# VISION-SJTU/UniDefense

Hardware: AMD Instinct MI355X
Metric: images/sec fwd+bwd (256x256, EffNet-b4) (higher is better)
Workload: dtype f32

## Files before the change

### include/unidefense_hip.h

```cpp
#ifndef UNIDEFENSE_HIP_H
#define UNIDEFENSE_HIP_H
#include <stdint.h>

#ifdef __cplusplus
extern "C" {
#endif

#define UD_EINVAL (-1000)

typedef void* ud_stream_t;

typedef struct {
    int N, Hin, Win, Cin, Hout, Wout, KH, KW, stride, pad_t, pad_l, transposed;
} ud_conv_geom;

typedef struct {
    const float* A; const float* B; float* C;
    int M, N, K;
    long lda, ldb, ldc;
    int a_mode, b_mode, out_mode, split_k;
    int batch; long strideA, strideB, strideC;
    ud_conv_geom g;
    double* stat_sum; double* stat_sumsq;
    int half_mask;
// ... 363 lines not shown
int ud_pw_bwd_fused_ok(int CE, int CIN);
int ud_pw_bwd_set_form(int form);
long ud_pw_bwd_fused_grid(long M);
int ud_pw_bwd_fused(const float* e, const float* dz, const ud_bn_ref* bn, const double* s1, const double* s2,
                    const double* s1_local, const double* s2_local, const float* x, const float* w, const float* add, long M,
                    int CE, int CIN, float* dx, float* dw, float* part, float* dgamma, float* dbeta, ud_stream_t stream);
int ud_pj_bwd_fused_ok(int CE, int CO, int HW);
int ud_pj_fwd_fused_ok(int CE, int CO, int HW);
int ud_pj_fwd_fused(const float* d, const ud_bn_ref* bn, const float* s, const float* w, int N, int HW, int CE, int CO, float* p,
                    double* sum, double* sumsq, ud_stream_t stream);
long ud_pj_bwd_fused_grid(int N, int HW, int CE, int CO);
int ud_mb_eval_dw_ok(int Ci, int CE, int K, int stride);
long ud_mb_eval_dw_tiles(int Ho, int Wo, int stride);
int ud_mb_eval_dw(const float* x, const float* we, const ud_bn_ref* bn0, const float* wt, const ud_bn_ref* bn1, float* d, float* part,
                  int N, int H, int W, int Ci, int CE, int Ho, int Wo, int K, int stride, int pad_t, int pad_l, int out_act,
                  ud_stream_t stream);
int ud_mb_eval_dw_h_ok(int Ci, int CE, int K, int stride);
long ud_mb_eval_dw_h_tiles(int Ho, int Wo, int stride);
int ud_mb_eval_dw_h(const void* x, const float* we, const ud_bn_ref* bn0, const float* wt, const ud_bn_ref* bn1, void* d, float* part,
                    int N, int H, int W, int Ci, int CE, int Ho, int Wo, int K, int stride, int pad_t, int pad_l, int out_act,
                    ud_stream_t stream);
int ud_pj_bwd_fused_a(const float* d, const float* dp, const ud_bn_ref* bn, const float* s, const float* w, int N, int HW, int CE,
                      int CO, float* dw, double* dgate, float* part, ud_stream_t stream);
int ud_pj_bwd_fused_b(const float* d, const float* dp, const ud_bn_ref* bn, const float* s, const float* dpool, float inv_hw,
                      const float* w, int N, int HW, int CE, int CO, float* dz, double* s1, double* s2, ud_stream_t stream);
int ud_normbwd_apply_plane_half(const void* x, const void* dy, const float* keep, float inv_keep, const ud_bn_ref* bn,
                                int dy_is_dz, const double* s1, const double* s2, const double* s1_local,
                                const double* s2_local, int G, int R, int C, uint16_t* plane, long panel_stride,
                                float* inv_scale, float* dgamma, float* dbeta, ud_stream_t stream);
int ud_se_bwd_a(const double* dgate, const float* s2, const float* s1, const float* We, double* ds1_acc, float* dWe,
                float* dbe, int N, int C, int Cs, ud_stream_t stream);
int ud_se_bwd_b(const double* ds1_acc, const float* s1, const float* Wr, const double* pool, float pool_scale,
                float* dpool, float* dWr, float* dbr, int N, int C, int Cs, ud_stream_t stream);
int ud_se_scale_bwd_bn(const void* dc, const void* x, const ud_bn_ref* bn, const float* s, const float* dpool,
    float inv_hw, void* dz, double* s1, double* s2, double* ws, int G, int R, int C, int f16, ud_stream_t
    stream);
long ud_coldot_bn_eval_ws_doubles(int G, int R, int C);
int ud_coldot_bn_eval(const void* dy, const void* x, const ud_bn_ref* bn, int G, int R, int C, double* out, double* ws,
                      int f16, ud_stream_t stream);
int ud_se_scale_bwd_bn_eval(const void* dc, const void* x, const ud_bn_ref* bn, const float* s, const float* dpool,
                            float inv_hw, void* dd, int G, int R, int C, int f16, ud_stream_t stream);
int ud_bn_eval_bwd(const void* dy, const void* x, const ud_bn_ref* bn, void* dx, int G, int R, int C, int f16,
                   ud_stream_t stream);
int ud_normbwd_apply_mix(const void* x, const void* dz, const ud_bn_ref* bn, const double* s1, const double* s2,
    const double* s1_local, const double* s2_local, const void* diff, int G, int R, int C, void* dd,
    double* dalpha_acc, float* dgamma, float* dbeta, double* energy, int f16, ud_stream_t stream);
int ud_gate_grad_from_acc(const double* acc, const float* alpha, float* out, ud_stream_t stream);
int ud_bn_apply(const void* x, const ud_bn_ref* bn, void* y, int G, int R, int C, int f16, ud_stream_t stream);
int ud_dwconv_bwd_data_bn(const void* dy, const float* gate_alpha, int gate_mode, const float* wt, const void*
    add, const void* x, const ud_bn_ref* bn, void* dz, double* s1, double* s2, double* ws, int N, int H, int W,
    int C, int Ho, int Wo, int K, int stride, int pad_t, int pad_l, int f16, ud_stream_t stream);
long ud_dwconv_bwd_data_bn_ws_doubles(int N, int H, int W, int C, int stride);
int ud_dwconv_bwd_data_ex(const void* dy, const float* gate_alpha, int gate_mode, const float* wt, const void*
    add, void* dx, int N, int H, int W, int C, int Ho, int Wo, int K, int stride, int pad_t, int pad_l, int f16,
    ud_stream_t stream);
int ud_dwconv_bwd_weight_ex(const void* x, const void* dy, const float* gate_alpha, int gate_mode, float* dwt,
    float* part, int chunks, int N, int H, int W, int C, int Ho, int Wo, int K, int stride, int pad_t, int
    pad_l, int f16, ud_stream_t stream);
int ud_rfft2_ex(const void* x, void* Y, int N, int S, int C, float scale, float w_interior, const ud_bn_ref* bn,
    void* act_out, const float* gate_alpha, int gate_mode, const double* gate_acc, float* gate_grad, int f16,
    uint32_t* absmax, ud_stream_t stream);
int ud_rfft2_ex_planes(const void* x, uint16_t* planes, long panel_stride, long plane_stride, float* inv_scale, float bound_pre,
                       const double* energy, int N, int S, int C, float scale, float w_interior, const ud_bn_ref* bn,
                       void* act_out, const float* gate_alpha, int gate_mode, const double* gate_acc, float* gate_grad,
                       const float* dw_wt, void* dw_out, int dw_k, ud_stream_t stream);
int ud_irfft2_mix(const void* Y, void* y, int N, int S, int C, float scale, float w_interior, const void* spat,
// ... 65 lines not shown
```

### unidefense_amd/csrc/fused.hip

```cpp
#include "bnref.h"

namespace {

struct Rows {
    int r, r_end;
    long idx, step;
};
__device__ __forceinline__ Rows rows_of(const RedGeom& q, int ri, int c4) {
    Rows w;
    const int g = blockIdx.z, p = blockIdx.x;
    const int r_begin = p * q.rows_per_chunk;
    w.r_end = r_begin + q.rows_per_chunk;
    if (w.r_end > q.R) w.r_end = q.R;
    w.step = (long)q.rpi * q.C4;
    w.r = r_begin + ri;
    w.idx = (long)g * q.R * q.C4 + (long)w.r * q.C4 + c4;
    return w;
}

__device__ __forceinline__ bool is_updater(int ri) { return blockIdx.x == 0 && blockIdx.z == 0 && ri == 0; }

template <int NQ>
__device__ __forceinline__ void red_out(const RedGeom& q, int ri, bool active, int c4, double (&v)[8], double* a1,
                                        double* a2, double* part, bool per_group) {
// ... 1217 lines not shown
                       (const _Float16*)nullptr, (_Float16*)nullptr, (double*)nullptr, dgamma, dbeta, (uint32_t*)nullptr,
                       (double*)nullptr, PlanesDst{plane, panel_stride, 0, inv_scale, nullptr});
    UD_LAUNCH_CHECK();
    return 0;
}

int ud_normbwd_apply_mix(const void* x, const void* dz, const ud_bn_ref* bn, const double* s1, const double* s2,
                         const double* s1_local, const double* s2_local, const void* diff, int G, int R, int C,
                         void* dd, double* dalpha_acc, float* dgamma, float* dbeta, double* energy, int f16,
                         ud_stream_t stream) {
    if (ud_bn_eval_form(bn)) return UD_EINVAL;
    if (!shape_ok(G, R, C) || !x || !dz || !bn || !s1 || !s2 || !dd || !diff || !dalpha_acc || bn->G != 1)
        return UD_EINVAL;
    if ((dgamma || dbeta) && (!s1_local || !s2_local)) return UD_EINVAL;
    RedGeom q = make_geom_ex(G, R, C, 512, 4096, 4);
    UD_STORAGE_DISPATCH(f16, hipLaunchKernelGGL((normbwd_apply_kernel<T, true>), red_grid(q), dim3(NT), 0,
                                                (hipStream_t)stream, q, (const T*)x, (const T*)dz, (const float*)nullptr,
                                                1.f, *bn, 1, s1, s2, s1_local, s2_local, (const T*)diff, (T*)dd,
                                                dalpha_acc, dgamma, dbeta, (uint32_t*)nullptr, energy,
                                                PlanesDst{nullptr, 0, 0, nullptr, nullptr}));
    UD_LAUNCH_CHECK();
    return 0;
}

int ud_gate_grad_from_acc(const double* acc, const float* alpha, float* out, ud_stream_t stream) {
    if (!acc || !alpha || !out) return UD_EINVAL;
    hipLaunchKernelGGL(gate_grad_from_acc_kernel, dim3(1), dim3(64), 0, (hipStream_t)stream, acc, alpha, out);
    UD_LAUNCH_CHECK();
    return 0;
}

int ud_se_bwd_a(const double* dgate, const float* s2, const float* s1, const float* We, double* ds1_acc, float* dWe,
                float* dbe, int N, int C, int Cs, ud_stream_t stream) {
    if (N < 1 || C < 1 || Cs < 1 || Cs > 128 || !dgate || !s2 || !s1 || !We || !ds1_acc || (!dWe != !dbe)) return UD_EINVAL;
    hipStream_t s = (hipStream_t)stream;
    const int role1 = N * ud_cdiv(C, Cs <= 64 ? 32 * (NT / 64) : 32 * (NT / 128));
    const bool wg = dWe != nullptr;
    if (Cs <= 64) {
        dim3 grid((unsigned)(role1 + (wg ? ud_cdiv(C, NT / 64) : 0)));
        hipLaunchKernelGGL(se_bwd_a_kernel<64>, grid, dim3(NT), 0, s, dgate, s2, s1, We, ds1_acc, dWe, dbe, N, C, Cs);
    } else {
        dim3 grid((unsigned)(role1 + (wg ? ud_cdiv(C, NT / 128) : 0)));
        hipLaunchKernelGGL(se_bwd_a_kernel<128>, grid, dim3(NT), 0, s, dgate, s2, s1, We, ds1_acc, dWe, dbe, N, C, Cs);
    }
    UD_LAUNCH_CHECK();
    return 0;
}

int ud_se_bwd_b(const double* ds1_acc, const float* s1, const float* Wr, const double* pool, float pool_scale,
                float* dpool, float* dWr, float* dbr, int N, int C, int Cs, ud_stream_t stream) {
    const bool wg = dWr != nullptr;
    if (N < 1 || N > NT || C < 1 || Cs < 1 || Cs > NT || !ds1_acc || !s1 || !Wr || !dpool || (!dWr != !dbr) || (wg && !pool))
        return UD_EINVAL;
    dim3 grid((unsigned)ud_cdiv(C, NT), (unsigned)(N + (wg ? Cs : 0)));
    hipLaunchKernelGGL(se_bwd_b_kernel, grid, dim3(NT), 0, (hipStream_t)stream, ds1_acc, s1, Wr, pool, pool_scale, dpool,
                       dWr, dbr, N, C, Cs);
    UD_LAUNCH_CHECK();
    return 0;
}

int ud_se_scale_bwd_bn(const void* dc, const void* x, const ud_bn_ref* bn, const float* s, const float* dpool,
                       float inv_hw, void* dz, double* s1, double* s2, double* ws, int G, int R, int C, int f16,
                       ud_stream_t stream) {
    if (ud_bn_eval_form(bn)) return UD_EINVAL;
    if (!shape_ok(G, R, C) || !dc || !x || !bn || !s || !dpool || !dz || !s1 || !s2 || bn->G != 1) return UD_EINVAL;
    hipStream_t st = (hipStream_t)stream;
    RedPlan pl = plan_reduce(G, R, C, false, ws);
    UD_STORAGE_DISPATCH(f16, hipLaunchKernelGGL(se_scale_bwd_bn_kernel<T>, red_grid(pl.q), dim3(NT), 0, st, pl.q,
                                                (const T*)dc, (const T*)x, *bn, s, dpool, inv_hw, (T*)dz, s1, s2,
                                                pl.use_part ? ws : nullptr));
    UD_LAUNCH_CHECK();
    return finish_reduce(pl, 2, false, C, ws, s1, s2, st);
}

static RedGeom coldot_eval_geom(int G, int R, int C) { return make_geom_ex(G, R, C, 1024, 64, 8); }

long ud_coldot_bn_eval_ws_doubles(int G, int R, int C) {
// ... 144 lines not shown
```

### unidefense_amd/kernels.py

```python
import ctypes as C
import math
import os

import torch

from . import lib as _lib
from .config import cfg as CFG
from .devmem import Scratch, ZeroPool
from .lib import ConvGeom, GemmDesc, GemmP3Desc

_call = _lib.call
_const, _rows = _lib.const, _lib.const_rows

GEMM_PROFILE = None


def _stream():
    return C.c_void_p(torch.cuda.current_stream().cuda_stream)


def _p(t):
    if t is None:
        return None
    return C.c_void_p(t.data_ptr())
# ... 2591 lines not shown
def se_scale_bn_planes(x, bn, s, G, R, amax):
    _chk(x, s)
    Cc = x.shape[-1]
    pl = Planes(G * R, Cc, x, 2, False)
    _call("ud_se_scale_bn_planes", _p(x), C.byref(bn.ref()), _p(s), _p(pl.buf), pl.panel, pl.plane, _p(pl.inv), _p(amax), G, R, Cc,
          _stream())
    return pl


def se_scale_bn_plane_half(x, bn, s, G, R):
    _act(x)
    _chk(s)
    Cc = x.shape[-1]
    pl = Planes(G * R, Cc, x, 1, False)
    _call("ud_se_scale_bn_plane_half", _p(x), C.byref(bn.ref()), _p(s), _p(pl.buf), pl.panel, _p(pl.inv), G, R, Cc, _stream())
    return pl


def coldot_bn(dy, x, bn, G, R, out):
    h = _act(dy, x)
    Cc = x.shape[-1]
    _call("ud_coldot_bn", _p(dy), _p(x), C.byref(bn.ref()), G, R, Cc, _pd(out), _fused_ws(x, G, R, Cc, True), h,
          _stream())


def fc_fwd_d(xsum, xscale, W, b, N):
    _chk(W, b)
    O, I = W.shape
    y = empty((N, O), W)
    _call("ud_fc_fwd_d", _pd(xsum), float(xscale), _p(W), _p(b), _p(y), N, I, O, _stream())
    return y


def bn_apply(x, bn, G, R, update=False):
    h = _act(x)
    y = torch.empty_like(x)
    _call("ud_bn_apply", _p(x), C.byref(bn.ref(update)), _p(y), G, R, x.shape[-1], h, _stream())
    return y


def se_scale_bn(x, bn, s, G, R, want_absmax=False):
    h = _act(x)
    _chk(s)
    y = torch.empty_like(x)
    amax = amax_slots(x, want_absmax)
    _call("ud_se_scale_bn", _p(x), C.byref(bn.ref()), _p(s), _p(y), G, R, x.shape[-1], h, _p(amax), _stream())
    y._ud_absmax = amax
    return y


def residual_bn(x, bn, keep, inv_keep, skip, G, R, update=False, want_absmax=False, planes_for=None):
    h = _act(x, skip)
    _chk(keep)
    out = torch.empty_like(x)
    amax = amax_slots(x, want_absmax)
    Cc = x.shape[-1]
    skip_amax = getattr(skip, "_ud_absmax", None) if skip is not None else None
    if (planes_for is not None and h == 0 and Cc % 4 == 0 and CFG.spectral_p2 != "off"
            and (skip is None or skip_amax is not None)
            and spectral_takes_planes(planes_for[0], planes_for[1], Cc, planes_for[2], want_stats=True)):
        pl = Planes(G * R, Cc, x, 2, False)
        _call("ud_residual_bn_planes", _p(x), C.byref(bn.ref(update)), _p(keep), float(inv_keep), _p(skip), _p(skip_amax), _p(out),
              _p(pl.buf), pl.panel, pl.plane, _p(pl.inv), G, R, Cc, _p(amax), _stream())
        out._ud_planes = pl
    else:
        _call("ud_residual_bn", _p(x), C.byref(bn.ref(update)), _p(keep), float(inv_keep), _p(skip), _p(out), G, R,
# ... 114 lines not shown


def project_bwd_fused_b(d, bn, s, dpool, inv_hw, dp2, w2, N, HW, sacc):
    _chk(d, dp2, w2, s, dpool)
    Co, Ce = w2.shape
    dz = torch.empty_like(d)
    _call("ud_pj_bwd_fused_b", _p(d), _p(dp2), C.byref(bn.ref()), _p(s), _p(dpool), float(inv_hw), _p(w2), N, HW, Ce, Co, _p(dz),
          _pd(sacc), _pd(sacc, Ce), _stream())
    return dz


def normbwd_apply_mix(x, dz, bn, G, R, sacc, diff, dalpha_acc, sacc_local=None, energy=None):
    h = _act(x, dz, diff)
    Cc = x.shape[-1]
    loc = sacc if sacc_local is None else sacc_local
    dd = torch.empty_like(x)
    dg = empty((Cc,), x)
    db = empty((Cc,), x)
    _call("ud_normbwd_apply_mix", _p(x), _p(dz), C.byref(bn.ref()), _pd(sacc), _pd(sacc, Cc), _pd(loc), _pd(loc, Cc),
          _p(diff), G, R, Cc, _p(dd), _pd(dalpha_acc), _p(dg), _p(db), _pd(energy) if energy is not None else None, h, _stream())
    return dd, dg, db


def gate_grad_from_acc(acc, alpha):
    out = empty((), alpha)
    _call("ud_gate_grad_from_acc", _pd(acc), _p(alpha), _p(out), _stream())
    return out


def se_bwd(dgate, s2, s1, We, Wr, pool, pool_scale, need_w=True):
    _chk(s2, s1, We, Wr)
    N, Cc = s2.shape
    Cs = s1.shape[1]
    ds1_acc = zeros64(N * Cs, s2)
    if not need_w:
        _call("ud_se_bwd_a", _pd(dgate), _p(s2), _p(s1), _p(We), _pd(ds1_acc), None, None, N, Cc, Cs, _stream())
        dpool = empty((N, Cc), s2)
        _call("ud_se_bwd_b", _pd(ds1_acc), _p(s1), _p(Wr), None, 0.0, _p(dpool), None, None, N, Cc, Cs, _stream())
        return dpool, None, None, None, None
    dWe = empty((Cc, Cs), s2)
    dbe = empty((Cc,), s2)
    _call("ud_se_bwd_a", _pd(dgate), _p(s2), _p(s1), _p(We), _pd(ds1_acc), _p(dWe), _p(dbe), N, Cc, Cs, _stream())
    dpool = empty((N, Cc), s2)
    dWr = empty((Cs, Cc), s2)
    dbr = empty((Cs,), s2)
    _call("ud_se_bwd_b", _pd(ds1_acc), _p(s1), _p(Wr), _pd(pool), float(pool_scale), _p(dpool), _p(dWr), _p(dbr), N, Cc,
          Cs, _stream())
    return dpool, dWe, dbe, dWr, dbr


def se_scale_bwd_bn(dc, x, bn, s, dpool, inv_hw, G, R, sacc):
    h = _act(dc, x)
    _chk(s, dpool)
    Cc = x.shape[-1]
    dz = torch.empty_like(x)
    _call("ud_se_scale_bwd_bn", _p(dc), _p(x), C.byref(bn.ref()), _p(s), _p(dpool), float(inv_hw), _p(dz), _pd(sacc),
          _pd(sacc, Cc), _fused_ws(x, G, R, Cc, False), G, R, Cc, h, _stream())
    return dz


def coldot_bn_eval(dy, x, bn, G, R, out):
    h = _act(dy, x)
    Cc = x.shape[-1]
    ws = _ws64(x, _call("ud_coldot_bn_eval_ws_doubles", G, R, Cc))
    _call("ud_coldot_bn_eval", _p(dy), _p(x), C.byref(bn.ref()), G, R, Cc, _pd(out), ws, h, _stream())

# ... 302 lines not shown
```

### unidefense_amd/mbconv.py

```python
import collections
from types import SimpleNamespace

import torch

from . import kernels as K
from . import tape as T
from .config import cfg


FUSED, HALF, EVAL_NODE, OPERATORS = "fused", "half", "eval_node", "operators"
TrunkMode = collections.namedtuple("TrunkMode", "kind wt dp", defaults=(None,))


_DW_TILED = True


_DW_TILE_OVERRIDE = {}
_DW_BWD_FUSED_OVERRIDE = {}


def _dw_tile_policy(sf, k, stride, H, half):
    ov = _DW_TILE_OVERRIDE.get((bool(sf), k, stride, H, bool(half)))
    if ov is not None and _DW_TILED:
        return ov
# ... 200 lines not shown
    if spat is None and t_fwd:
        spat = K.dwtile_fwd(src, wt, k, g.pt, g.pl, g.Ho, g.Wo, bn=src_bn, stride=stride)
    elif spat is None:
        spat = K.dwconv_fwd(a, wt, k, stride, g.pt, g.pl, g.Ho, g.Wo)
    b.a = a
    b.xf_shape = (g.N, S, S // 2 + 1, 2 * Ce)
    if isinstance(xf, K.Planes):
        yf, b.sctx = K.spectral_fwd(xf, g.Wf)
    else:
        yf, b.sctx = K.spectral_fwd(xf.view(-1, 2 * Ce), g.Wf, x_absmax=getattr(xf, "_ud_absmax", None))
    yf = yf.view(b.xf_shape)
    xf = None
    if stride == 1:
        b.d, b.fr = K.irfft2_mix(yf, g.s_i, spat, g.alpha, acc1)
        spat = None
    else:
        b.fr = K.irfft2(yf, g.s_i, 1.0)
        b.d = K.sfmix_fwd(spat, b.fr, g.alpha, True)
        K.colstats(b.d.view(g.Mo, Ce), acc1)
        b.spat = spat
    del yf


def _fwd_se(b):
    g, x, blk, d = b.geo, b.x, b.blk, b.d
    b.pool = K.zeros64(g.N * g.Ce, x)
    b.c_pl = (d.dtype == torch.float32 and g.Ce % 32 == 0 and cfg.spectral_p2 != "off"
              and K.spectral_takes_planes(g.Mo, g.Co, g.Ce, g.Wp, want_stats=True))
    c_amax = None
    if b.c_pl:
        c_amax = K.colsum_bn_amax(d, b.bn1, g.N, g.HWo, b.pool, update=True)
    else:
        K.colsum_bn(d, b.bn1, g.N, g.HWo, b.pool, update=True)
    b.s1 = K.fc_fwd_d(b.pool, 1.0 / g.HWo, g.Wsr, blk._se_reduce.bias, g.N)
    b.s2 = K.fc_fwd(b.s1, g.Wse, blk._se_expand.bias, 1)
    return c_amax


def _fwd_project(b, c_amax, next_blk):
    g, x, blk, d, bn1, s2 = b.geo, b.x, b.blk, b.d, b.bn1, b.s2
    acc2 = K.zeros64(2 * g.Co, x)
    if not b.c_pl and K.project_fwd_fused_ok(d, g.Wp, g.HWo):
        p, b.pctx = K.project_fwd_fused(d, bn1, s2, g.Wp, g.N, g.HWo, stats=acc2)
        done = True
    elif b.c_pl:
        c = K.se_scale_bn_planes(d, bn1, s2, g.N, g.HWo, c_amax)
        (p, done), b.pctx = K.spectral_fwd(c, g.Wp, stats=acc2)
    elif (d.dtype == torch.float16 and g.Ce % 8 == 0 and K.spectral_takes_plane_half(g.Mo, g.Co, g.Ce)):
        c = K.se_scale_bn_plane_half(d, bn1, s2, g.N, g.HWo)
        (p, done), b.pctx = K.spectral_fwd(c, g.Wp, stats=acc2)
    else:
        c = K.se_scale_bn(d, bn1, s2, g.N, g.HWo, want_absmax=True)
        (p, done), b.pctx = K.spectral_fwd(c.view(g.Mo, g.Ce), g.Wp, stats=acc2, x_absmax=getattr(c, "_ud_absmax", None))
    if not done:
        K.colstats(p, acc2)
    b.dp.reduce(acc2)
    b.bn2 = _bn_of(blk._bn2, acc2, g.Mo * b.dp.world, 0)
    b.p4 = p.view(g.N, g.Ho, g.Wo, g.Co)
    nxt = None
    if next_blk is not None and next_blk.spec.expand != 1:
        nxt = (g.Mo, next_blk.spec.cexp, next_blk._expand_conv.weight.view(next_blk.spec.cexp, g.Co))
    b.out = K.residual_bn(b.p4, b.bn2, b.keep, b.inv_keep, x if blk.spec.skip else None, g.N, g.HWo, update=True, want_absmax=True, planes_for=nxt)


def _fused_backward(b, tape):
    dout = tape.pop_grad(b.out)
    if dout is None:
        return
# ... 142 lines not shown
    if thin:
        dx, dWe, dg0, db0 = _expand_dgrad(tape, skip, dout, x, lambda acc: K.expand_bwd_fused(e, dz0, b.bn0, sb0, loc0, ectx.x, ectx.w, add=acc))
    else:
        de2, de_amax, dg0, db0 = _normbwd_to_gemm(ectx, gr.de_pl, e, dz0, None, 1.0, b.bn0, gr.is_dz, 1, g.M, sb0, loc0)
    tape.add_param_grad(blk._bn0.weight, dg0)
    tape.add_param_grad(blk._bn0.bias, db0)
    if not thin:
        dx, dWe = _expand_dgrad(tape, skip, dout, x, lambda acc: K.spectral_bwd(ectx, de2, out=acc, dy_absmax=de_amax))
    tape.add_param_grad(blk._expand_conv.weight, dWe)
    return dx


def _half_forward(x, blk, g, wt, src_bn):
    bn1 = K.EvalBN(blk._bn1, 1)
    if g.We is not None:
        src, src_bn = K.gemm_nt(x.view(g.M, g.Cin), g.We).view(g.N, g.H, g.W, g.Ce), K.EvalBN(blk._bn0, 1)
    else:
        src = x
    spat = K.dwtile_fwd(src, wt, g.k, g.pt, g.pl, g.Ho, g.Wo, bn=src_bn, stride=g.stride)
    xf_shape = None
    if g.sf:
        xf, _ = K.rfft2_ex(src, g.s_f, 1.0, bn=src_bn)
        xf_shape = xf.shape
        yf = K.gemm_nt(xf.view(-1, 2 * g.Ce), g.Wf).view(xf_shape)
        if g.stride == 1:
            d, _ = K.irfft2_mix(yf, g.s_i, spat, g.alpha, None)
        else:
            d = K.sfmix_fwd(spat, K.irfft2(yf, g.s_i, 1.0), g.alpha, True)
        del xf, yf, spat
    else:
        d = spat
    pool = K.zeros64(g.N * g.Ce, x)
    K.colsum_bn(d, bn1, g.N, g.HWo, pool)
    s1 = K.fc_fwd_d(pool, 1.0 / g.HWo, g.Wsr, blk._se_reduce.bias, g.N)
    out, s2, bn2 = _eval_half_tail(x, blk, g, d, bn1, s1)
    return out, SimpleNamespace(src=src, src_bn=src_bn, d=d, s1=s1, s2=s2, bn1=bn1, bn2=bn2, xf_shape=xf_shape)


def _eval_half_tail(x, blk, g, d, bn1, s1):
    s2 = K.fc_fwd(s1, g.Wse, blk._se_expand.bias, 1)
    p = K.gemm_nt(K.se_scale_bn(d, bn1, s2, g.N, g.HWo).view(g.Mo, g.Ce), g.Wp)
    bn2 = K.EvalBN(blk._bn2, 0)
    return K.residual_bn(p.view(g.N, g.Ho, g.Wo, g.Co), bn2, None, 1.0, x if blk.spec.skip else None, g.N, g.HWo), s2, bn2


def mbconv_eval_half(x, blk, wt, lazy_bn=None, node_max_cin=0):
    sp = blk.spec
    g = block_geom(blk, x)
    assert x.dtype == torch.float16 and not (sp.skip and lazy_bn is not None)
    if (sp.expand != 1 and sp.sf_norm is None and g.Cin <= node_max_cin and K.mb_eval_dw_h_ok(g.Cin, g.Ce, g.k, g.stride)):
        bn1 = K.EvalBN(blk._bn1, 1)
        d, pmean = K.mb_eval_dw_h(x, g.We, K.EvalBN(blk._bn0, 1), wt, bn1, g.k, g.stride, g.pt, g.pl, g.Ho, g.Wo, out_act=False)
        s1 = K.fc_fwd(pmean, g.Wsr, blk._se_reduce.bias, 0)
        return _eval_half_tail(x, blk, g, d, bn1, s1)[0]
    return _half_forward(x, blk, g, wt, lazy_bn)[0]


HALF_GRAD_PROBE = None


def mbconv_frozen_half(tape, x, blk, wt, lazy_in=None):
    if tape.wgrad_on:
        raise RuntimeError("mbconv_frozen_half is the backward of a FROZEN model (no parameter requires a gradient): it forms no "
                           "weight gradient; a half-storage backward with trainable parameters is the training step's")
    assert x.dtype == torch.float16 and not (blk.spec.skip and lazy_in is not None)
    g = block_geom(blk, x)
    out, f = _half_forward(x, blk, g, wt, lazy_in.bn if lazy_in is not None else None)
    tape.record(lambda: _frozen_backward(tape, x, blk, g, wt, lazy_in, out, f))
    return out


def _frozen_backward(tape, x, blk, g, wt, lazy_in, out, f):
    dout = tape.pop_grad(out)
    if dout is None:
        return
    dout = _grad_like(dout, out)
    assert dout.dtype == torch.float16
    skip, d, N, HWo = blk.spec.skip, f.d, g.N, g.HWo
    probe = HALF_GRAD_PROBE
    dp = K.bn_eval_bwd(dout, None, f.bn2, 1, g.Mo)
    dc = K.gemm_nn(dp.view(g.Mo, g.Co), g.Wp).view(N, g.Ho, g.Wo, g.Ce)
    if probe is not None:
        for nm, t in (("dout", dout), ("dp", dp), ("dc", dc)):
            probe(blk, nm, t)
    dgate = K.zeros64(N * g.Ce, x)
    K.coldot_bn_eval(dc, d, f.bn1, N, HWo, dgate)
    dpool = K.se_bwd(dgate, f.s2, f.s1, g.Wse, g.Wsr, None, 1.0 / HWo, need_w=False)[0]
# ... 11 lines not shown
            for nm, t in (("dyf", dyf), ("dxf", dxf), ("da_f", da_f)):
                probe(blk, nm, t)
        del dfr, dyf, dxf
        g_alpha, g_mode = g.alpha, 2
    if f.src_bn is not None:
        de = K.dwtile_dgrad_eval(dd, wt, g.k, g.pt, g.pl, f.src, f.src_bn, g_alpha, g_mode, da_f, g.stride)
        if probe is not None:
            probe(blk, "de", de)
        if lazy_in is not None:
            lazy_in.backward(de)
            return
        dx, = _expand_dgrad(tape, skip, dout, x, lambda acc: (K.gemm_nn(de.view(g.M, g.Ce), g.We, out=acc, accumulate=acc is not None),))
    else:
        add, skip_done = _skip_into_add(skip, da_f, dout)
        dx = K.dwtile_bwd_data(dd, wt, g.k, g.pt, g.pl, g.H, g.W, g_alpha, g_mode, add, stride=g.stride)
        if not skip_done:
            dx = K.axpby(dx, 1.0, dout, 1.0, out=dx)
    if probe is not None:
        probe(blk, "dx", dx)
    dx._ud_owned = True
    tape.add_grad(x, dx)


def eval_block_ok(blk, max_cin):
    sp = blk.spec
    return (sp.expand != 1 and sp.sf_norm is None and sp.cin <= max_cin and K.mb_eval_dw_ok(sp.cin, sp.cexp, sp.k, sp.stride))


def mbconv_eval(x, blk, wt):
    g = block_geom(blk, x)
    bn1 = K.EvalBN(blk._bn1, 1)
    pj = K.project_fwd_fused_ok(x, g.Wp, g.HWo)
    d, pool = K.mb_eval_dw(x, g.We, K.EvalBN(blk._bn0, 1), wt, bn1, g.k, g.stride, g.pt, g.pl, g.Ho, g.Wo, out_act=not pj)
    s1 = K.fc_fwd(pool, g.Wsr, blk._se_reduce.bias, 0)
    s2 = K.fc_fwd(s1, g.Wse, blk._se_expand.bias, 1)
    if pj:
        p, _ = K.project_fwd_fused(d, bn1, s2, g.Wp, g.N, g.HWo)
    else:
        p = K.gemm_nt(K.se_scale_fwd(d, s2).view(g.Mo, g.Ce), g.Wp)
    return K.residual_bn(p.view(g.N, g.Ho, g.Wo, g.Co), K.EvalBN(blk._bn2, 0), None, 1.0, x if blk.spec.skip else None, g.N, g.HWo)
```

Measured before the change: 1439.

## Fuse SE reduce/expand FCs into one kernel forward and one kernel backward

Adds a fused squeeze-excite kernel that runs the reduce FC, swish and expand FC in a single launch, keeping the pooled vector and hidden activations in LDS. A fused backward kernel computes dpool and all four weight and bias gradients in one multi-role launch, replacing the two-stage ud_se_bwd_a/ud_se_bwd_b path and its float64 accumulation buffer. The aim is to cut launch count and the global round trips for the small SE tensors in every MBConv block. Each path is gated by size heuristics on C*Cs and N*C and falls back to the old kernels otherwise. The generalised se_bwd_a template for Cs above 128 adds code paths with little coverage.

```diff
diff --git a/include/unidefense_hip.h b/include/unidefense_hip.h
--- a/include/unidefense_hip.h
+++ b/include/unidefense_hip.h
@@ -419,6 +419,13 @@
                 float* dbe, int N, int C, int Cs, ud_stream_t stream);
 int ud_se_bwd_b(const double* ds1_acc, const float* s1, const float* Wr, const double* pool, float pool_scale,
                 float* dpool, float* dWr, float* dbr, int N, int C, int Cs, ud_stream_t stream);
+#define UD_SE_FC_MAX_C 4096
+#define UD_SE_FC_MAX_CS 128
+int ud_se_fc_fwd(const double* pool_sum, float pool_scale, const float* pool_mean, const float* Wr, const float* br,
+                 const float* We, const float* be, float* s1, float* s2, int N, int C, int Cs, ud_stream_t stream);
+int ud_se_fc_bwd(const double* dgate, const float* s2, const float* s1, const float* We, const float* Wr,
+                 const double* pool, float pool_scale, float* dpool, float* dWe, float* dbe, float* dWr, float* dbr, int N,
+                 int C, int Cs, ud_stream_t stream);
 int ud_se_scale_bwd_bn(const void* dc, const void* x, const ud_bn_ref* bn, const float* s, const float* dpool,
     float inv_hw, void* dz, double* s1, double* s2, double* ws, int G, int R, int C, int f16, ud_stream_t
     stream);
diff --git a/unidefense_amd/csrc/fused.hip b/unidefense_amd/csrc/fused.hip
--- a/unidefense_amd/csrc/fused.hip
+++ b/unidefense_amd/csrc/fused.hip
@@ -1273,17 +1273,18 @@
 
 int ud_se_bwd_a(const double* dgate, const float* s2, const float* s1, const float* We, double* ds1_acc, float* dWe,
                 float* dbe, int N, int C, int Cs, ud_stream_t stream) {
-    if (N < 1 || C < 1 || Cs < 1 || Cs > 128 || !dgate || !s2 || !s1 || !We || !ds1_acc || (!dWe != !dbe)) return UD_EINVAL;
+    if (N < 1 || C < 1 || Cs < 1 || Cs > NT || !dgate || !s2 || !s1 || !We || !ds1_acc || (!dWe != !dbe)) return UD_EINVAL;
     hipStream_t s = (hipStream_t)stream;
-    const int role1 = N * ud_cdiv(C, Cs <= 64 ? 32 * (NT / 64) : 32 * (NT / 128));
+    const int ip = Cs <= 64 ? 64 : (Cs <= 128 ? 128 : NT);
+    const int role1 = N * ud_cdiv(C, 32 * (NT / ip));
     const bool wg = dWe != nullptr;
-    if (Cs <= 64) {
-        dim3 grid((unsigned)(role1 + (wg ? ud_cdiv(C, NT / 64) : 0)));
+    dim3 grid((unsigned)(role1 + (wg ? ud_cdiv(C, NT / ip) : 0)));
+    if (ip == 64)
         hipLaunchKernelGGL(se_bwd_a_kernel<64>, grid, dim3(NT), 0, s, dgate, s2, s1, We, ds1_acc, dWe, dbe, N, C, Cs);
-    } else {
-        dim3 grid((unsigned)(role1 + (wg ? ud_cdiv(C, NT / 128) : 0)));
+    else if (ip == 128)
         hipLaunchKernelGGL(se_bwd_a_kernel<128>, grid, dim3(NT), 0, s, dgate, s2, s1, We, ds1_acc, dWe, dbe, N, C, Cs);
-    }
+    else
+        hipLaunchKernelGGL(se_bwd_a_kernel<NT>, grid, dim3(NT), 0, s, dgate, s2, s1, We, ds1_acc, dWe, dbe, N, C, Cs);
     UD_LAUNCH_CHECK();
     return 0;
 }
diff --git a/unidefense_amd/csrc/sefc.hip b/unidefense_amd/csrc/sefc.hip
--- /dev/null
+++ b/unidefense_amd/csrc/sefc.hip
@@ -0,0 +1,387 @@
+#include "ud_common.h"
+
+namespace {
+
+constexpr int NTS = 1024;
+constexpr int NW = NTS / 64;
+constexpr int MAXC = UD_SE_FC_MAX_C;
+constexpr int MAXCS = UD_SE_FC_MAX_CS;
+constexpr int KU = 16;
+static_assert(MAXC % (64 * KU) == 0 && MAXCS <= NTS / 8, "the padded trip counts and the LDS carves below assume these");
+constexpr int KUR = 4;
+constexpr int RU = 2;
+constexpr int NR = 64;
+
+__device__ __forceinline__ float dpre_at(const double* dgate, const float* s2, long i) {
+    const float g = ud_sigmoid_fast(s2[i]);
+    return (float)dgate[i] * g * (1.f - g);
+}
+
+template <bool WAVE_OUT>
+__global__ __launch_bounds__(NTS) void se_fc_fwd_kernel(const double* __restrict__ xsum, float xscale,
+                                                        const float* __restrict__ xmean, const float* __restrict__ Wr,
+                                                        const float* __restrict__ br, const float* __restrict__ We,
+                                                        const float* __restrict__ be, float* __restrict__ s1,
+                                                        float* __restrict__ s2, int C, int Cs, int span) {
+    __shared__ float sx[MAXC];
+    __shared__ float sh[MAXCS];
+    const int n = blockIdx.y, tid = threadIdx.x, lane = tid & 63, wave = tid >> 6;
+    const int KP = ((C + 63) / 64 + KU - 1) / KU * KU;
+    for (int c = tid; c < KP * 64; c += NTS)
+        sx[c] = c < C ? (xsum ? (float)xsum[(long)n * C + c] * xscale : xmean[(long)n * C + c]) : 0.f;
+    __syncthreads();
+    for (int i = wave; i < Cs; i += 2 * NW) {
+        const bool two = i + NW < Cs;
+        const float* w0 = Wr + (long)i * C;
+        const float* w1 = Wr + (long)(two ? i + NW : i) * C;
+        float acc0 = 0.f, acc1 = 0.f;
+        for (int k0 = 0; k0 < KP; k0 += KU) {
+            float wv0[KU], wv1[KU];
+#pragma unroll
+            for (int j = 0; j < KU; ++j) {
+                const int cc = min(lane + 64 * (k0 + j), C - 1);
+                wv0[j] = w0[cc];
+                wv1[j] = w1[cc];
+            }
+#pragma unroll
+            for (int j = 0; j < KU; ++j) {
+                const float xv = sx[lane + 64 * (k0 + j)];
+                acc0 += xv * wv0[j];
+                acc1 += xv * wv1[j];
+            }
+        }
+        acc0 = ud_wave_sum(acc0);
+        acc1 = ud_wave_sum(acc1);
+        if (lane < 2 && (lane == 0 || two)) {
+            const int iu = i + lane * NW;
+            const float v = (lane ? acc1 : acc0) + (br ? br[iu] : 0.f);
+            sh[iu] = ud_swish(v);
+            if (blockIdx.x == 0) s1[(long)n * Cs + iu] = v;
+        }
+    }
+    __syncthreads();
+    const int o_end = min(C, ((int)blockIdx.x + 1) * span);
+    if (WAVE_OUT) {
+        for (int o = blockIdx.x * span + wave; o < o_end; o += NW) {
+            float acc = 0.f;
+#pragma unroll 4
+            for (int i = lane; i < Cs; i += 64) acc += sh[i] * We[(long)o * Cs + i];
+            acc = ud_wave_sum(acc);
+            if (lane == 0) s2[(long)n * C + o] = acc + (be ? be[o] : 0.f);
+        }
+        return;
+    }
+    for (int o = blockIdx.x * span + tid; o < o_end; o += NTS) {
+        const float* w = We + (long)o * Cs;
+        float acc = 0.f;
+        if ((Cs & 3) == 0) {
+#pragma unroll 8
+            for (int i = 0; i < Cs; i += 4) {
+                const f32x4 v = *reinterpret_cast<const f32x4*>(w + i);
+                acc += sh[i] * v[0] + sh[i + 1] * v[1] + sh[i + 2] * v[2] + sh[i + 3] * v[3];
+            }
+        } else {
+#pragma unroll 4
+            for (int i = 0; i < Cs; ++i) acc += sh[i] * w[i];
+        }
+        s2[(long)n * C + o] = acc + (be ? be[o] : 0.f);
+    }
+}
+
+constexpr int LDS_BWD = MAXC + 4 * NTS + 16 * MAXCS + MAXCS;
+
+__global__ __launch_bounds__(NTS) void se_fc_bwd_kernel(const double* __restrict__ dgate, const float* __restrict__ s2,
+                                                        const float* __restrict__ s1, const float* __restrict__ We,
+                                                        const float* __restrict__ Wr, const double* __restrict__ pool,
+                                                        float pool_scale, float* __restrict__ dpool,
+                                                        float* __restrict__ dWe, float* __restrict__ dbe,
+                                                        float* __restrict__ dWr, float* __restrict__ dbr, int N, int C,
+                                                        int Cs, int G, int span, int EB) {
+    __shared__ float lds[LDS_BWD];
+    const int tid = threadIdx.x, lane = tid & 63, wave = tid >> 6;
+    int b = blockIdx.x;
+    if (b < N * G) {
+        float* dp = lds;
+        float* part = lds + MAXC;
+        float* part2 = part + 4 * NTS;
+        float* ds = part2 + 16 * MAXCS;
+        const int n = b / G, g = b % G;
+        constexpr int PW = 8;
+        const int c0 = g * span, cn = min(span, C - c0);
+        const int SL = min(min(NTS / span, Cs), 16);
+        const int cl = tid % span, sl = tid / span;
+        const bool pooler = sl < SL && cl < cn, pre = (Cs + SL - 1) / SL <= PW;
+        const float s1v = tid < Cs ? s1[(long)n * Cs + tid] : 0.f;
+        float wv[PW];
+#pragma unroll
+        for (int j = 0; j < PW; ++j) {
+            const int i = sl + j * SL;
+            wv[j] = (pooler && pre && i < Cs) ? Wr[(long)i * C + c0 + cl] : 0.f;
+        }
+        for (int c = tid; c < C; c += NTS) dp[c] = dpre_at(dgate, s2, (long)n * C + c);
+        __syncthreads();
+        const int V = (Cs & 3) ? 1 : 4, Q = Cs / V, R = NTS / Q;
+        const int q = tid % Q, r = tid / Q;
+        if (r < R) {
+            const int TP = ((C + R - 1) / R + 7) / 8 * 8;
+            if (V == 4) {
+                f32x4 a = {0.f, 0.f, 0.f, 0.f};
+                for (int t0 = 0; t0 < TP; t0 += 8) {
+                    f32x4 v[8];
+                    float d[8];
+#pragma unroll
+                    for (int j = 0; j < 8; ++j) {
+                        const int c = r + (t0 + j) * R, cc = min(c, C - 1);
+                        v[j] = *reinterpret_cast<const f32x4*>(We + (long)cc * Cs + 4 * q);
+                        d[j] = c < C ? dp[cc] : 0.f;
+                    }
+#pragma unroll
+                    for (int j = 0; j < 8; ++j) a += d[j] * v[j];
+                }
+                *reinterpret_cast<f32x4*>(part + r * Cs + 4 * q) = a;
+            } else {
+                float a = 0.f;
+                for (int t0 = 0; t0 < TP; t0 += 8) {
+                    float v[8], d[8];
+#pragma unroll
+                    for (int j = 0; j < 8; ++j) {
+                        const int c = r + (t0 + j) * R, cc = min(c, C - 1);
+                        v[j] = We[(long)cc * Cs + q];
+                        d[j] = c < C ? dp[cc] : 0.f;
+                    }
+#pragma unroll
+                    for (int j = 0; j < 8; ++j) a += d[j] * v[j];
+                }
+                part[r * Cs + q] = a;
+            }
+        }
+        __syncthreads();
+        const int H = min(NTS / Cs, 16);
+        {
+            const int i = tid % Cs, h = tid / Cs;
+            if (h < H) {
+                float s = 0.f;
+                for (int rr = h; rr < R; rr += H) s += part[rr * Cs + i];
+                part2[h * Cs + i] = s;
+            }
+        }
+        __syncthreads();
+        if (tid < Cs) {
+            float s = 0.f;
+            for (int h = 0; h < H; ++h) s += part2[h * Cs + tid];
+            ds[tid] = s * ud_act_grad_fast(s1v, 1);
+        }
+        __syncthreads();
+        if (pooler) {
+            float a = 0.f;
+            if (pre) {
+#pragma unroll
+                for (int j = 0; j < PW; ++j) a += (sl + j * SL < Cs ? ds[sl + j * SL] : 0.f) * wv[j];
+            } else {
+                const float* w = Wr + c0 + cl;
+#pragma unroll 8
+                for (int i = sl; i < Cs; i += SL) a += ds[i] * w[(long)i * C];
+            }
+            part[sl * span + cl] = a;
+        }
+        __syncthreads();
+        if (tid < cn) {
+            float s = 0.f;
+            for (int k = 0; k < SL; ++k) s += part[k * span + tid];
+            dpool[(long)n * C + c0 + tid] = s;
+        }
+        return;
+    }
+    b -= N * G;
+    if (b < EB) {
+        float* sh = lds;
+        const int IP = Cs <= 64 ? 64 : 128, NSL = NTS / IP;
+        const int i = tid % IP, sl = tid / IP;
+        const int c = b * NSL + sl;
+        const bool own = c < C && i < Cs;
+        float acc = 0.f, accb = 0.f;
+        for (int n0 = 0; n0 < N; n0 += IP) {
+            const int nn = min(IP, N - n0);
+            __syncthreads();
+            sh[sl * IP + i] = (c < C && i < nn) ? dpre_at(dgate, s2, (long)(n0 + i) * C + c) : 0.f;
+            __syncthreads();
+            if (own) {
+                for (int nb = 0; nb < nn; nb += 16) {
+                    float sv[16];
+#pragma unroll
+                    for (int j = 0; j < 16; ++j) sv[j] = s1[(long)(n0 + min(nb + j, nn - 1)) * Cs + i];
+#pragma unroll
+                    for (int j = 0; j < 16; ++j) {
+                        if (nb + j < nn) {
+                            const float gn = sh[sl * IP + nb + j];
+                            acc += gn * ud_act_fast(sv[j], 1);
+                            accb += gn;
+                        }
+                    }
+                }
+            }
+        }
+        if (!own) return;
+        dWe[(long)c * Cs + i] = acc;
+        if (i == 0) dbe[c] = accb;
+        return;
+    }
+    b -= EB;
+    {
+        float* wI = lds;
+        float* dsl = lds + RU * MAXC;
+        const int i0 = b * RU;
+        const bool has1 = i0 + 1 < Cs;
+        for (int c = tid; c < C; c += NTS) {
+            wI[RU * c] = We[(long)c * Cs + i0];
+            wI[RU * c + 1] = has1 ? We[(long)c * Cs + i0 + 1] : 0.f;
+        }
+        const int KP = ((C + 63) / 64 + KUR - 1) / KUR * KUR;
+        const int CT = min(NTS, (C + 63) / 64 * 64), SN = NTS / CT;
+        const int cl = tid % CT, sn = tid / CT;
+        float acc[MAXC / NTS][RU] = {};
+        float bsum = 0.f;
+        for (int n0 = 0; n0 < N; n0 += NR) {
+            const int nn = min(NR, N - n0);
+            __syncthreads();
+            for (int nl = wave; nl < nn; nl += 2 * NW) {
+                const bool two = nl + NW < nn;
+                const int nl2 = two ? nl + NW : nl;
+                const long base0 = (long)(n0 + nl) * C, base1 = (long)(n0 + nl2) * C;
+                const float* sp0 = s1 + (long)(n0 + nl) * Cs + i0;
+                const float* sp1 = s1 + (long)(n0 + nl2) * Cs + i0;
+                const float s1v[2][RU] = {{sp0[0], has1 ? sp0[1] : 0.f}, {sp1[0], has1 ? sp1[1] : 0.f}};
+                float a[2][RU] = {};
+                for (int k0 = 0; k0 < KP; k0 += KUR) {
+                    double dg[2][KUR];
+                    float sv[2][KUR];
+#pragma unroll
+                    for (int j = 0; j < KUR; ++j) {
+                        const int cc = min(lane + 64 * (k0 + j), C - 1);
+                        dg[0][j] = dgate[base0 + cc];
+                        sv[0][j] = s2[base0 + cc];
+                        dg[1][j] = dgate[base1 + cc];
+                        sv[1][j] = s2[base1 + cc];
+                    }
+#pragma unroll
+                    for (int j = 0; j < KUR; ++j) {
+                        const int c = lane + 64 * (k0 + j), cc = min(c, C - 1);
+                        const float w0 = c < C ? wI[RU * cc] : 0.f, w1 = c < C ? wI[RU * cc + 1] : 0.f;
+#pragma unroll
+                        for (int u = 0; u < 2; ++u) {
+                            const float gs = ud_sigmoid_fast(sv[u][j]);
+                            const float d = (float)dg[u][j] * gs * (1.f - gs);
+                            a[u][0] += d * w0;
+                            a[u][1] += d * w1;
+                        }
+                    }
+                }
+#pragma unroll
+                for (int u = 0; u < 2; ++u) {
+                    a[u][0] = ud_wave_sum(a[u][0]);
+                    a[u][1] = ud_wave_sum(a[u][1]);
+                }
+                if (lane < 2 && (lane == 0 || two)) {
+                    const int u = lane, nlu = u ? nl2 : nl;
+                    dsl[RU * nlu] = (u ? a[1][0] : a[0][0]) * ud_act_grad_fast(u ? s1v[1][0] : s1v[0][0], 1);
+                    dsl[RU * nlu + 1] = has1 ? (u ? a[1][1] : a[0][1]) * ud_act_grad_fast(u ? s1v[1][1] : s1v[0][1], 1) : 0.f;
+                }
+            }
+            __syncthreads();
+            if (tid < RU)
+                for (int nl = 0; nl < nn; ++nl) bsum += dsl[RU * nl + tid];
+            if (CT < NTS) {
+                if (sn < SN && cl < C) {
+#pragma unroll 8
+                    for (int nl = sn; nl < nn; nl += SN) {
+                        const float p = (float)pool[(long)(n0 + nl) * C + cl] * pool_scale;
+                        acc[0][0] += dsl[RU * nl] * p;
+                        acc[0][1] += dsl[RU * nl + 1] * p;
+                    }
+                }
+            } else {
+#pragma unroll 4
+                for (int nl = sn; nl < nn; nl += SN) {
+                    const double* pr = pool + (long)(n0 + nl) * C;
+                    const float d0 = dsl[RU * nl], d1 = dsl[RU * nl + 1];
+#pragma unroll
+                    for (int m = 0; m < MAXC / NTS; ++m) {
+                        const int c = cl + m * CT;
+                        const float p = c < C ? (float)pr[c] * pool_scale : 0.f;
+                        acc[m][0] += d0 * p;
+                        acc[m][1] += d1 * p;
+                    }
+                }
+            }
+        }
+        if (SN > 1) {
+            __syncthreads();
+            if (sn < SN) {
+                wI[(sn * CT + cl) * RU] = acc[0][0];
+                wI[(sn * CT + cl) * RU + 1] = acc[0][1];
+            }
+            __syncthreads();
+            if (sn == 0) {
+                acc[0][0] = acc[0][1] = 0.f;
+                for (int k = 0; k < SN; ++k) {
+                    acc[0][0] += wI[(k * CT + cl) * RU];
+                    acc[0][1] += wI[(k * CT + cl) * RU + 1];
+                }
+            }
+        }
+        if (sn == 0) {
+#pragma unroll
+            for (int m = 0; m < MAXC / NTS; ++m) {
+                const int c = cl + m * CT;
+                if (c < C) {
+                    dWr[(long)i0 * C + c] = acc[m][0];
+                    if (has1) dWr[(long)(i0 + 1) * C + c] = acc[m][1];
+                }
+            }
+        }
+        if (tid < RU && i0 + tid < Cs) dbr[i0 + tid] = bsum;
+    }
+}
+
+inline int clampi(int v, int lo, int hi) { return v < lo ? lo : (v > hi ? hi : v); }
+inline bool se_fc_range_ok(int N, int C, int Cs) { return N >= 1 && N <= 65535 && C >= 1 && C <= MAXC && Cs >= 1 && Cs <= MAXCS; }
+
+}
+
+int ud_se_fc_fwd(const double* pool_sum, float pool_scale, const float* pool_mean, const float* Wr, const float* br,
+                 const float* We, const float* be, float* s1, float* s2, int N, int C, int Cs, ud_stream_t stream) {
+    if (!se_fc_range_ok(N, C, Cs) || (!pool_sum == !pool_mean) || !Wr || !We || !s1 || !s2) return UD_EINVAL;
+    const bool wave_out = C < 256;
+    int G = clampi(ud_cdiv(C, wave_out ? NW : 64), 1, 256 / N > 1 ? 256 / N : 1);
+    const int span = ud_cdiv(C, G);
+    G = ud_cdiv(C, span);
+    dim3 grid((unsigned)G, (unsigned)N);
+    if (wave_out)
+        hipLaunchKernelGGL(se_fc_fwd_kernel<true>, grid, dim3(NTS), 0, (hipStream_t)stream, pool_sum, pool_scale, pool_mean, Wr,
+                           br, We, be, s1, s2, C, Cs, span);
+    else
+        hipLaunchKernelGGL(se_fc_fwd_kernel<false>, grid, dim3(NTS), 0, (hipStream_t)stream, pool_sum, pool_scale, pool_mean, Wr,
+                           br, We, be, s1, s2, C, Cs, span);
+    UD_LAUNCH_CHECK();
+    return 0;
+}
+
+int ud_se_fc_bwd(const double* dgate, const float* s2, const float* s1, const float* We, const float* Wr,
+                 const double* pool, float pool_scale, float* dpool, float* dWe, float* dbe, float* dWr, float* dbr, int N,
+                 int C, int Cs, ud_stream_t stream) {
+    const bool wg = dWe != nullptr;
+    if (!se_fc_range_ok(N, C, Cs) || !dgate || !s2 || !s1 || !We || !Wr || !dpool || (!dbe != !wg) || (!dWr != !wg) ||
+        (!dbr != !wg) || (wg && !pool))
+        return UD_EINVAL;
+    const int gmin = ud_cdiv(C, NTS);
+    int G = clampi(ud_cdiv(C, 128), gmin, 256 / N > gmin ? 256 / N : gmin);
+    const int span = ud_cdiv(C, G);
+    G = ud_cdiv(C, span);
+    const int EB = wg ? ud_cdiv(C, NTS / (Cs <= 64 ? 64 : 128)) : 0, RB = wg ? ud_cdiv(Cs, RU) : 0;
+    const long blocks = (long)N * G + EB + RB;
+    if (blocks > 0x7fffffffL) return UD_EINVAL;
+    hipLaunchKernelGGL(se_fc_bwd_kernel, dim3((unsigned)blocks), dim3(NTS), 0, (hipStream_t)stream, dgate, s2, s1, We, Wr, pool,
+                       pool_scale, dpool, dWe, dbe, dWr, dbr, N, C, Cs, G, span, EB);
+    UD_LAUNCH_CHECK();
+    return 0;
+}
diff --git a/unidefense_amd/kernels.py b/unidefense_amd/kernels.py
--- a/unidefense_amd/kernels.py
+++ b/unidefense_amd/kernels.py
@@ -2647,6 +2647,40 @@
     return y
 
 
+SE_FC_MAX_C, SE_FC_MAX_CS = _const("UD_SE_FC_MAX_C"), _const("UD_SE_FC_MAX_CS")
+
+
+SE_FC_FWD_MAX_W = 20480
+SE_FC_WGRAD_MAX_NC = 6144
+
+
+def _se_fc_ok(N, Cc, Cs):
+    return 1 <= N <= 65535 and 1 <= Cc <= SE_FC_MAX_C and 1 <= Cs <= SE_FC_MAX_CS
+
+
+def se_fc_fwd_pays(N, Cc, Cs):
+    return _se_fc_ok(N, Cc, Cs) and Cc * Cs <= SE_FC_FWD_MAX_W
+
+
+def se_fc_bwd_pays(N, Cc, Cs, need_w):
+    return need_w and _se_fc_ok(N, Cc, Cs) and N * Cc <= SE_FC_WGRAD_MAX_NC
+
+
+def se_fc_fwd(pool, pool_scale, Wr, br, We, be, N):
+    _chk(Wr, br, We, be)
+    Cs, Cc = Wr.shape
+    sums = pool.dtype == torch.float64
+    if not sums:
+        _chk(pool)
+    if not se_fc_fwd_pays(N, Cc, Cs):
+        s1 = fc_fwd_d(pool, pool_scale, Wr, br, N) if sums else fc_fwd(pool.view(N, Cc), Wr, br, 0)
+        return s1, fc_fwd(s1, We, be, 1)
+    s1, s2 = empty((N, Cs), Wr), empty((N, Cc), Wr)
+    _call("ud_se_fc_fwd", _pd(pool) if sums else None, float(pool_scale) if sums else 0.0, None if sums else _p(pool), _p(Wr),
+          _p(br), _p(We), _p(be), _p(s1), _p(s2), N, Cc, Cs, _stream())
+    return s1, s2
+
+
 def bn_apply(x, bn, G, R, update=False):
     h = _act(x)
     y = torch.empty_like(x)
@@ -2827,6 +2861,12 @@
     _chk(s2, s1, We, Wr)
     N, Cc = s2.shape
     Cs = s1.shape[1]
+    if se_fc_bwd_pays(N, Cc, Cs, need_w):
+        dpool = empty((N, Cc), s2)
+        dWe, dbe, dWr, dbr = empty((Cc, Cs), s2), empty((Cc,), s2), empty((Cs, Cc), s2), empty((Cs,), s2)
+        _call("ud_se_fc_bwd", _pd(dgate), _p(s2), _p(s1), _p(We), _p(Wr), _pd(pool), float(pool_scale), _p(dpool), _p(dWe),
+              _p(dbe), _p(dWr), _p(dbr), N, Cc, Cs, _stream())
+        return dpool, dWe, dbe, dWr, dbr
     ds1_acc = zeros64(N * Cs, s2)
     if not need_w:
         _call("ud_se_bwd_a", _pd(dgate), _p(s2), _p(s1), _p(We), _pd(ds1_acc), None, None, N, Cc, Cs, _stream())
diff --git a/unidefense_amd/mbconv.py b/unidefense_amd/mbconv.py
--- a/unidefense_amd/mbconv.py
+++ b/unidefense_amd/mbconv.py
@@ -256,8 +256,7 @@
         c_amax = K.colsum_bn_amax(d, b.bn1, g.N, g.HWo, b.pool, update=True)
     else:
         K.colsum_bn(d, b.bn1, g.N, g.HWo, b.pool, update=True)
-    b.s1 = K.fc_fwd_d(b.pool, 1.0 / g.HWo, g.Wsr, blk._se_reduce.bias, g.N)
-    b.s2 = K.fc_fwd(b.s1, g.Wse, blk._se_expand.bias, 1)
+    b.s1, b.s2 = K.se_fc_fwd(b.pool, 1.0 / g.HWo, g.Wsr, blk._se_reduce.bias, g.Wse, blk._se_expand.bias, g.N)
     return c_amax
 
 
@@ -466,16 +465,15 @@
         d = spat
     pool = K.zeros64(g.N * g.Ce, x)
     K.colsum_bn(d, bn1, g.N, g.HWo, pool)
-    s1 = K.fc_fwd_d(pool, 1.0 / g.HWo, g.Wsr, blk._se_reduce.bias, g.N)
-    out, s2, bn2 = _eval_half_tail(x, blk, g, d, bn1, s1)
+    s1, s2 = K.se_fc_fwd(pool, 1.0 / g.HWo, g.Wsr, blk._se_reduce.bias, g.Wse, blk._se_expand.bias, g.N)
+    out, bn2 = _eval_half_tail(x, blk, g, d, bn1, s2)
     return out, SimpleNamespace(src=src, src_bn=src_bn, d=d, s1=s1, s2=s2, bn1=bn1, bn2=bn2, xf_shape=xf_shape)
 
 
-def _eval_half_tail(x, blk, g, d, bn1, s1):
-    s2 = K.fc_fwd(s1, g.Wse, blk._se_expand.bias, 1)
+def _eval_half_tail(x, blk, g, d, bn1, s2):
     p = K.gemm_nt(K.se_scale_bn(d, bn1, s2, g.N, g.HWo).view(g.Mo, g.Ce), g.Wp)
     bn2 = K.EvalBN(blk._bn2, 0)
-    return K.residual_bn(p.view(g.N, g.Ho, g.Wo, g.Co), bn2, None, 1.0, x if blk.spec.skip else None, g.N, g.HWo), s2, bn2
+    return K.residual_bn(p.view(g.N, g.Ho, g.Wo, g.Co), bn2, None, 1.0, x if blk.spec.skip else None, g.N, g.HWo), bn2
 
 
 def mbconv_eval_half(x, blk, wt, lazy_bn=None, node_max_cin=0):
@@ -485,8 +483,8 @@
     if (sp.expand != 1 and sp.sf_norm is None and g.Cin <= node_max_cin and K.mb_eval_dw_h_ok(g.Cin, g.Ce, g.k, g.stride)):
         bn1 = K.EvalBN(blk._bn1, 1)
         d, pmean = K.mb_eval_dw_h(x, g.We, K.EvalBN(blk._bn0, 1), wt, bn1, g.k, g.stride, g.pt, g.pl, g.Ho, g.Wo, out_act=False)
-        s1 = K.fc_fwd(pmean, g.Wsr, blk._se_reduce.bias, 0)
-        return _eval_half_tail(x, blk, g, d, bn1, s1)[0]
+        s2 = K.se_fc_fwd(pmean, None, g.Wsr, blk._se_reduce.bias, g.Wse, blk._se_expand.bias, g.N)[1]
+        return _eval_half_tail(x, blk, g, d, bn1, s2)[0]
     return _half_forward(x, blk, g, wt, lazy_bn)[0]
 
 
@@ -564,8 +562,7 @@
     bn1 = K.EvalBN(blk._bn1, 1)
     pj = K.project_fwd_fused_ok(x, g.Wp, g.HWo)
     d, pool = K.mb_eval_dw(x, g.We, K.EvalBN(blk._bn0, 1), wt, bn1, g.k, g.stride, g.pt, g.pl, g.Ho, g.Wo, out_act=not pj)
-    s1 = K.fc_fwd(pool, g.Wsr, blk._se_reduce.bias, 0)
-    s2 = K.fc_fwd(s1, g.Wse, blk._se_expand.bias, 1)
+    s2 = K.se_fc_fwd(pool, None, g.Wsr, blk._se_reduce.bias, g.Wse, blk._se_expand.bias, g.N)[1]
     if pj:
         p, _ = K.project_fwd_fused(d, bn1, s2, g.Wp, g.N, g.HWo)
     else:
```

Result: no change. 1438, median of 2 (-0.1%).
